# samiazirar/mvtracker

Hardware: AMD Instinct MI355X
Metric: query-points*frames/sec, 4-view 24-frame 512x512 @1024 queries (higher is better)
Workload: dtype bf16; 1 GPU; c3: 4-view synthetic 24-frame 512x512, 1024 queries, bf16 (configs[2], the metric's config); 4-view 24-frame 512x512, 1024 queries per GPU, corr K=16 x 4 levels, iters=4, 3 windows, random-init weights (seeded recipe); queries_total=1024, parallelism=query-shard x1, frame_store=bf16 rows

## Files before the change

mvtracker_amd/csrc/attention_mfma.hip:

```cpp
#include "common.h"

namespace {

typedef __bf16 bf16x8 __attribute__((ext_vector_type(8)));
typedef __bf16 bf16x4 __attribute__((ext_vector_type(4)));
typedef unsigned u32x2 __attribute__((ext_vector_type(2)));
typedef unsigned u32x4 __attribute__((ext_vector_type(4)));

constexpr int DH = 48;
constexpr int LDV = 40;

__device__ __forceinline__ bf16x8 load8(const float* base, long long off, int bf) {
  if (bf) return __builtin_bit_cast(bf16x8, *reinterpret_cast<const u32x4*>(reinterpret_cast<const unsigned short*>(base) + off));
  const float* p = base + off;
  const f32x4 a = *reinterpret_cast<const f32x4*>(p), b = *reinterpret_cast<const f32x4*>(p + 4);
  const bf16x4 x = __builtin_convertvector(a, bf16x4), y = __builtin_convertvector(b, bf16x4);
  bf16x8 o;
#pragma unroll
  for (int e = 0; e < 4; ++e) {
    o[e] = x[e];
    o[4 + e] = y[e];
  }
  return o;
}

template <int KS, bool BFIN>
__device__ __forceinline__ void attention_mfma(const float* __restrict__ q, int ldq, long long q_gs, long long q_is,
                                               const float* __restrict__ k, const float* __restrict__ v, int ldkv, long long k_gs,
                                               long long k_is, float* __restrict__ o, int ldo, int groups, int nq, int nk, int heads,
                                               int bf_out, float* __restrict__ ws, unsigned bx, unsigned by, unsigned gx, unsigned gy) {
  constexpr int bf_in = BFIN ? 1 : 0;
  constexpr int NW = KS == 1 ? 4 : KS;
  constexpr int VT = 64 * LDV;
  constexpr int MERGE = KS > 1 ? (KS - 1) * 64 * 68 : 0;
  __shared__ __attribute__((aligned(16))) unsigned short vts[NW * VT];
  __shared__ float red[MERGE > 0 ? MERGE : 1];
  const int lane = threadIdx.x & 63;
  const int wave = __builtin_amdgcn_readfirstlane(threadIdx.x >> 6);
  const int r = lane & 31, h = lane >> 5;
  unsigned short* vt = vts + wave * VT;

  const int chunks = (nq + 63) / 64;
  const long long nchunk = (long long)groups * heads * chunks;
  unsigned bxl = bx, byl = by;
#ifndef MVT_ATTN_NO_XCD
  if (KS > 1 && ws) {
    const unsigned total = gx * gy;
    if (total % 8 == 0) {
      const unsigned L = bx + gx * by;
      const unsigned V = (L % 8) * (total / 8) + L / 8;
      bxl = V / gy;
      byl = V % gy;
    }
  }
#endif
  const long long chunk_id = KS == 1 ? (long long)bxl * 4 + wave : (long long)bxl;
  const bool chunk_ok = chunk_id < nchunk;
  const long long cid = chunk_ok ? chunk_id : 0;
  const int qc = (int)(cid % chunks);
  const int hd = (int)((cid / chunks) % heads);
  const long long g = cid / ((long long)chunks * heads);

  const int nkb = (nk + 31) / 32;
  const int gper = ws ? (nkb + (int)gy - 1) / (int)gy : nkb;
  const int g0 = ws ? (int)byl * gper : 0;
  const int g1 = g0 + gper < nkb ? g0 + gper : nkb;
  const int per = (gper + KS - 1) / KS;
  const int kb0 = KS == 1 ? g0 : g0 + wave * per;
  const int kb1 = KS == 1 ? g1 : (kb0 + per < g1 ? kb0 + per : g1);
  const long long kvbase = (g * k_gs) * ldkv + hd * DH;
  const long long kstep = k_is * ldkv;
  struct KV {
    bf16x8 kf[3];
    f32x4 vraw[6];
  };
  auto load_kv = [&](int kb, KV& t) {
    const int key = kb * 32 + r;
    const long long ko = kvbase + (long long)(key < nk ? key : nk - 1) * kstep;
#pragma unroll
    for (int ks = 0; ks < 3; ++ks) t.kf[ks] = load8(k, ko + ks * 16 + 8 * h, bf_in);
    const long long vo = ko + 24 * h;
#pragma unroll
    for (int i = 0; i < 6; ++i) {
      if (bf_in) {
        const uint2 w = *reinterpret_cast<const uint2*>(reinterpret_cast<const unsigned short*>(v) + vo + 4 * i);
        t.vraw[i] = (f32x4){__uint_as_float(w.x), __uint_as_float(w.y), 0.f, 0.f};
      } else {
        t.vraw[i] = *reinterpret_cast<const f32x4*>(v + vo + 4 * i);
      }
    }
  };
  KV cur;
  if (kb0 < kb1) load_kv(kb0, cur);

  const float scale = 1.0f / sqrtf((float)DH);
  bf16x8 qf[2][3];
#pragma unroll
  for (int mb = 0; mb < 2; ++mb) {
    const int qi = qc * 64 + mb * 32 + r;
    const long long qo = (g * q_gs + (long long)(qi < nq ? qi : nq - 1) * q_is) * ldq + hd * DH;
#pragma unroll
    for (int ks = 0; ks < 3; ++ks) {
      f32x4 a = load_act4(q, qo + ks * 16 + 8 * h, bf_in), b = load_act4(q, qo + ks * 16 + 8 * h + 4, bf_in);
#pragma unroll
      for (int e = 0; e < 4; ++e) {
        a[e] *= scale;
        b[e] *= scale;
      }
      const bf16x4 x = __builtin_convertvector(a, bf16x4), y = __builtin_convertvector(b, bf16x4);
#pragma unroll
      for (int e = 0; e < 4; ++e) {
        qf[mb][ks][e] = x[e];
        qf[mb][ks][4 + e] = y[e];
      }
    }
  }
  for (int i = lane; i < 16 * LDV; i += 64) vt[48 * LDV + i] = 0;
  __builtin_amdgcn_fence(__ATOMIC_SEQ_CST, "wavefront");

  f32x16 oacc[2][2];
  float m[2], l[2];
#pragma unroll
  for (int mb = 0; mb < 2; ++mb) {
    m[mb] = -INFINITY;
    l[mb] = 0.f;
#pragma unroll
    for (int db = 0; db < 2; ++db)
#pragma unroll
      for (int e = 0; e < 16; ++e) oacc[mb][db][e] = 0.f;
  }

#pragma unroll 1
  for (int kb = kb0; kb < kb1; ++kb) {
    KV nxt = cur;
    if (kb + 1 < kb1) load_kv(kb + 1, nxt);
    const int key = kb * 32 + r;
    bf16x8 kf[3];
#pragma unroll
    for (int ks = 0; ks < 3; ++ks) kf[ks] = cur.kf[ks];
    {
      __builtin_amdgcn_fence(__ATOMIC_SEQ_CST, "wavefront");
#pragma unroll
      for (int i = 0; i < 6; ++i) {
        f32x4 a = cur.vraw[i];
        if (bf_in) {
          const unsigned wx = __float_as_uint(a[0]), wy = __float_as_uint(a[1]);
          a = (f32x4){__uint_as_float(wx << 16), __uint_as_float(wx & 0xFFFF0000u), __uint_as_float(wy << 16), __uint_as_float(wy & 0xFFFF0000u)};
        }
        if (key >= nk) a = (f32x4){0.f, 0.f, 0.f, 0.f};
        const u32x2 w = __builtin_bit_cast(u32x2, __builtin_convertvector(a, bf16x4));
#pragma unroll
        for (int e = 0; e < 4; ++e) vt[(24 * h + 4 * i + e) * LDV + r] = (unsigned short)((e & 1) ? (w[e >> 1] >> 16) : (w[e >> 1] & 0xFFFFu));
      }
      __builtin_amdgcn_fence(__ATOMIC_SEQ_CST, "wavefront");
    }
#pragma unroll
    for (int mb = 0; mb < 2; ++mb) {
      f32x16 s;
#pragma unroll
      for (int e = 0; e < 16; ++e) s[e] = 0.f;
#pragma unroll
      for (int ks = 0; ks < 3; ++ks) s = __builtin_amdgcn_mfma_f32_32x32x16_bf16(kf[ks], qf[mb][ks], s, 0, 0, 0);
      float mx = -INFINITY;
#pragma unroll
      for (int e = 0; e < 16; ++e) {
        const int kk = kb * 32 + (e & 3) + 8 * (e >> 2) + 4 * h;
        if (kk >= nk) s[e] = -INFINITY;
        mx = fmaxf(mx, s[e]);
      }
      mx = fmaxf(mx, __shfl_xor(mx, 32, 64));
      const float mn = fmaxf(m[mb], mx);
      const float corr = (m[mb] == -INFINITY) ? 0.f : __expf(m[mb] - mn);
      float ps = 0.f;
#pragma unroll
      for (int e = 0; e < 16; ++e) {
        s[e] = __expf(s[e] - mn);
        ps += s[e];
      }
      l[mb] = l[mb] * corr + ps;
      m[mb] = mn;
      if (__ballot(corr != 1.0f)) {
#pragma unroll
        for (int db = 0; db < 2; ++db)
#pragma unroll
          for (int e = 0; e < 16; ++e) oacc[mb][db][e] *= corr;
      }
#pragma unroll
      for (int sk = 0; sk < 2; ++sk) {
        f32x4 lo4, hi4;
#pragma unroll
        for (int e = 0; e < 4; ++e) {
          lo4[e] = s[8 * sk + e];
          hi4[e] = s[8 * sk + 4 + e];
        }
        const bf16x4 bl = __builtin_convertvector(lo4, bf16x4), bh = __builtin_convertvector(hi4, bf16x4);
        bf16x8 pb;
#pragma unroll
        for (int e = 0; e < 4; ++e) {
          pb[e] = bl[e];
          pb[4 + e] = bh[e];
        }
#pragma unroll
        for (int db = 0; db < 2; ++db) {
          const unsigned short* vr = &vt[(db * 32 + r) * LDV + 16 * sk + 4 * h];
          const u32x2 a0 = *reinterpret_cast<const u32x2*>(vr), a1 = *reinterpret_cast<const u32x2*>(vr + 8);
          const bf16x8 va = __builtin_bit_cast(bf16x8, (u32x4){a0[0], a0[1], a1[0], a1[1]});
          oacc[mb][db] = __builtin_amdgcn_mfma_f32_32x32x16_bf16(va, pb, oacc[mb][db], 0, 0, 0);
        }
      }
    }
    cur = nxt;
  }

  if (KS > 1) {
    if (wave > 0) {
      float* rr = red + ((wave - 1) * 64 + lane) * 68;
#pragma unroll
      for (int mb = 0; mb < 2; ++mb) {
        rr[mb] = m[mb];
        rr[2 + mb] = l[mb];
#pragma unroll
        for (int db = 0; db < 2; ++db)
#pragma unroll
          for (int e = 0; e < 16; ++e) rr[4 + (mb * 2 + db) * 16 + e] = oacc[mb][db][e];
      }
    }
    __syncthreads();
    if (wave > 0) return;
#pragma unroll 1
    for (int w = 0; w < KS - 1; ++w) {
      const float* rr = red + (w * 64 + lane) * 68;
#pragma unroll
      for (int mb = 0; mb < 2; ++mb) {
        const float mw = rr[mb];
        const float mn = fmaxf(m[mb], mw);
        const float ca = (m[mb] == -INFINITY) ? 0.f : __expf(m[mb] - mn);
        const float cb = (mw == -INFINITY) ? 0.f : __expf(mw - mn);
        l[mb] = fmaf(l[mb], ca, rr[2 + mb] * cb);
#pragma unroll
        for (int db = 0; db < 2; ++db)
#pragma unroll
          for (int e = 0; e < 16; ++e) oacc[mb][db][e] = fmaf(oacc[mb][db][e], ca, rr[4 + (mb * 2 + db) * 16 + e] * cb);
        m[mb] = mn;
      }
    }
  }
  if (!chunk_ok) return;
  if (ws) {
    {
      const long long rec = byl * nchunk + chunk_id;
      *reinterpret_cast<f32x4*>(ws + mvt_part_off(rec, 0, lane)) = (f32x4){m[0], m[1], l[0], l[1]};
#pragma unroll
      for (int mb = 0; mb < 2; ++mb)
#pragma unroll
        for (int db = 0; db < 2; ++db)
#pragma unroll
          for (int gq = 0; gq < 4; ++gq)
            *reinterpret_cast<f32x4*>(ws + mvt_part_off(rec, 1 + (mb * 2 + db) * 4 + gq, lane)) =
                (f32x4){oacc[mb][db][4 * gq], oacc[mb][db][4 * gq + 1], oacc[mb][db][4 * gq + 2], oacc[mb][db][4 * gq + 3]};
    }
    return;
  }
#pragma unroll
  for (int mb = 0; mb < 2; ++mb) {
    const float lt = l[mb] + __shfl_xor(l[mb], 32, 64);
    const float inv = 1.0f / lt;
    const int qi = qc * 64 + mb * 32 + r;
    if (qi >= nq) continue;
    const long long oo = (g * q_gs + (long long)qi * q_is) * ldo + hd * DH;
#pragma unroll
    for (int db = 0; db < 2; ++db) {
#pragma unroll
      for (int gq = 0; gq < 4; ++gq) {
        const int d = db * 32 + 8 * gq + 4 * h;
        if (d < DH) {
          f32x4 t;
#pragma unroll
          for (int e = 0; e < 4; ++e) t[e] = oacc[mb][db][4 * gq + e] * inv;
          store_act4(o, oo + d, t, bf_out);
        }
      }
    }
  }
}

__device__ __forceinline__ void attention_merge(const float* __restrict__ ws, int nsplit, long long nchunk, long long q_gs, long long q_is,
                                                float* __restrict__ o, int ldo, int nq, int heads, int bf_out, long long bid) {
  const int lane = threadIdx.x & 63;
  const long long cid = bid * 4 + (threadIdx.x >> 6);
  if (cid >= nchunk) return;
  const int r = lane & 31, h = lane >> 5;
  const int chunks = (nq + 63) / 64;
  const int qc = (int)(cid % chunks);
  const int hd = (int)((cid / chunks) % heads);
  const long long g = cid / ((long long)chunks * heads);
  float m[2], l[2];
  f32x16 oacc[2][2];
  auto ld = [&](long long rec, int quad) { return *reinterpret_cast<const f32x4*>(ws + mvt_part_off(rec, quad, lane)); };
  {
    const f32x4 q0 = ld(cid, 0);
#pragma unroll
    for (int mb = 0; mb < 2; ++mb) {
      m[mb] = q0[mb];
      l[mb] = q0[2 + mb];
#pragma unroll
      for (int db = 0; db < 2; ++db)
#pragma unroll
        for (int gq = 0; gq < 4; ++gq) {
          const f32x4 t = ld(cid, 1 + (mb * 2 + db) * 4 + gq);
#pragma unroll
          for (int e = 0; e < 4; ++e) oacc[mb][db][4 * gq + e] = t[e];
        }
    }
  }
#pragma unroll 1
  for (int w = 1; w < nsplit; ++w) {
    const long long rec = w * nchunk + cid;
    const f32x4 q0 = ld(rec, 0);
#pragma unroll
    for (int mb = 0; mb < 2; ++mb) {
      const float mw = q0[mb];
      const float mn = fmaxf(m[mb], mw);
      const float ca = (m[mb] == -INFINITY) ? 0.f : __expf(m[mb] - mn);
      const float cb = (mw == -INFINITY) ? 0.f : __expf(mw - mn);
      l[mb] = fmaf(l[mb], ca, q0[2 + mb] * cb);
#pragma unroll
      for (int db = 0; db < 2; ++db)
#pragma unroll
        for (int gq = 0; gq < 4; ++gq) {
          const f32x4 t = ld(rec, 1 + (mb * 2 + db) * 4 + gq);
#pragma unroll
          for (int e = 0; e < 4; ++e) oacc[mb][db][4 * gq + e] = fmaf(oacc[mb][db][4 * gq + e], ca, t[e] * cb);
        }
      m[mb] = mn;
    }
  }
#pragma unroll
  for (int mb = 0; mb < 2; ++mb) {
    const float lt = l[mb] + __shfl_xor(l[mb], 32, 64);
    const float inv = 1.0f / lt;
    const int qi = qc * 64 + mb * 32 + r;
    if (qi >= nq) continue;
    const long long oo = (g * q_gs + (long long)qi * q_is) * ldo + hd * DH;
#pragma unroll
    for (int db = 0; db < 2; ++db) {
#pragma unroll
      for (int gq = 0; gq < 4; ++gq) {
        const int d = db * 32 + 8 * gq + 4 * h;
        if (d < DH) {
          f32x4 t;
#pragma unroll
          for (int e = 0; e < 4; ++e) t[e] = oacc[mb][db][4 * gq + e] * inv;
          store_act4(o, oo + d, t, bf_out);
        }
      }
    }
  }
}

#define ATTN_ARGS                                                                                                               \
  const float *__restrict__ q, int ldq, long long q_gs, long long q_is, const float *__restrict__ k, const float *__restrict__ v, \
      int ldkv, long long k_gs, long long k_is, float *__restrict__ o, int ldo, int groups
template <int KS, bool BFIN>
__global__ __launch_bounds__(KS == 1 ? 256 : KS * 64) void attention_mfma_kernel(ATTN_ARGS, int nq, int nk, int heads, int bf_in_unused,
                                                                                int bf_out, float* __restrict__ ws) {
  attention_mfma<KS, BFIN>(q, ldq, q_gs, q_is, k, v, ldkv, k_gs, k_is, o, ldo, groups, nq, nk, heads, bf_out, ws, blockIdx.x, blockIdx.y,
                           gridDim.x, gridDim.y);
}
__global__ __launch_bounds__(256) void attention_merge_kernel(const float* __restrict__ ws, int nsplit, long long nchunk, long long q_gs,
                                                              long long q_is, float* __restrict__ o, int ldo, int nq, int heads,
                                                              int bf_out) {
  attention_merge(ws, nsplit, nchunk, q_gs, q_is, o, ldo, nq, heads, bf_out, blockIdx.x);
}

__device__ __forceinline__ const float* row_ptr(const float* base, long long r, int ld, int bf) {
  return bf ? reinterpret_cast<const float*>(reinterpret_cast<const unsigned short*>(base) + r * ld) : base + r * ld;
}

template <int KS, bool BFIN>
__global__ __launch_bounds__(KS == 1 ? 256 : KS * 64) void attention_mfma_seg_kernel(ATTN_ARGS, int heads, int bf_out,
                                                                                    float* __restrict__ ws, mvt_seg_table t) {
  const int s = mvt_seg_find(t, blockIdx.x);
  const int bf = BFIN ? 1 : 0;
  attention_mfma<KS, BFIN>(row_ptr(q, t.qrow[s], ldq, bf), ldq, q_gs, q_is, row_ptr(k, t.krow[s], ldkv, bf), row_ptr(v, t.krow[s], ldkv, bf),
                           ldkv, k_gs, k_is, const_cast<float*>(row_ptr(o, t.qrow[s], ldo, bf_out)), ldo, groups, t.nq[s], t.nk[s], heads,
                           bf_out, ws ? ws + t.ws[s] : nullptr, (unsigned)(blockIdx.x - t.blk[s]), blockIdx.y,
                           (unsigned)(t.blk[s + 1] - t.blk[s]), gridDim.y);
}
__global__ __launch_bounds__(256) void attention_merge_seg_kernel(const float* __restrict__ ws, int nsplit, int groups, long long q_gs,
                                                                  long long q_is, float* __restrict__ o, int ldo, int heads, int bf_out,
                                                                  mvt_seg_table t) {
  const int s = mvt_seg_find(t, blockIdx.x);
  const long long nchunk = (long long)groups * heads * ((t.nq[s] + 63) / 64);
  attention_merge(ws + t.ws[s], nsplit, nchunk, q_gs, q_is, const_cast<float*>(row_ptr(o, t.qrow[s], ldo, bf_out)), ldo, t.nq[s], heads,
                  bf_out, blockIdx.x - t.blk[s]);
}
#undef ATTN_ARGS

}

extern "C" int mvt_attention_bf16(const void* q, int ldq, long long q_gs, long long q_is, const void* k, const void* v,
                                  int ldkv, long long k_gs, long long k_is, void* o, int ldo, int groups, int nq, int nk,
                                  int heads, int dh, int io_flags, float* workspace, void* stream) {
  MVT_REQUIRE((io_flags & ~(MVT_IO_IN_BF16 | MVT_IO_OUT_BF16 | MVT_ATTN_PARTIALS_ONLY)) == 0);
  const bool partials_only = (io_flags & MVT_ATTN_PARTIALS_ONLY) != 0;
  const int bf_in = io_flags & MVT_IO_IN_BF16 ? 1 : 0, bf_out = io_flags & MVT_IO_OUT_BF16 ? 1 : 0;
  MVT_REQUIRE(!bf_in || (ldq % 8 == 0 && ldkv % 8 == 0));
  MVT_REQUIRE(!bf_out || ldo % 8 == 0);
  MVT_REQUIRE(q && k && v && o && groups > 0 && nq > 0 && nk > 0 && heads > 0 && dh == DH);
  MVT_REQUIRE(ldq % 4 == 0 && ldkv % 4 == 0 && ldo % 4 == 0 && ldq >= heads * dh && ldkv >= heads * dh && ldo >= heads * dh);
  MVT_REQUIRE(((uintptr_t)q % 16 == 0) && ((uintptr_t)k % 16 == 0) && ((uintptr_t)v % 16 == 0) && ((uintptr_t)o % 16 == 0));
  const long long nchunk = (long long)groups * heads * ((nq + 63) / 64);
#define LAUNCH_T(KS, BF, BLOCKS, THREADS, WSP)                                                                                        \
  hipLaunchKernelGGL((attention_mfma_kernel<KS, BF>), BLOCKS, dim3(THREADS), 0, mvt_stream(stream), (const float*)q, ldq, q_gs, q_is, \
                     (const float*)k, (const float*)v, ldkv, k_gs, k_is, (float*)o, ldo, groups, nq, nk, heads, bf_in, bf_out, WSP)
#define LAUNCH(KS, BLOCKS, THREADS)                                         \
  do {                                                                      \
    if (bf_in) LAUNCH_T(KS, true, dim3((unsigned)(BLOCKS)), THREADS, WS);  \
    else LAUNCH_T(KS, false, dim3((unsigned)(BLOCKS)), THREADS, WS);       \
  } while (0)
  constexpr int NSPLIT = MVT_ATTN_NSPLIT;
  MVT_REQUIRE(!partials_only || (nk >= 512 && nchunk < 256 && workspace && ((nk + 31) / 32) % NSPLIT == 0));
  if (nk >= 512 && nchunk < 256 && workspace && ((nk + 31) / 32) % NSPLIT == 0) {
    MVT_REQUIRE((uintptr_t)workspace % 16 == 0);
#define WS workspace
    if (bf_in) LAUNCH_T(4, true, dim3((unsigned)nchunk, NSPLIT), 256, workspace);
    else LAUNCH_T(4, false, dim3((unsigned)nchunk, NSPLIT), 256, workspace);
#undef WS
    if (!partials_only)
      hipLaunchKernelGGL(attention_merge_kernel, dim3((unsigned)mvt_cdiv(nchunk, 4)), dim3(256), 0, mvt_stream(stream), workspace, NSPLIT,
                         nchunk, q_gs, q_is, (float*)o, ldo, nq, heads, bf_out);
    return mvt_launch_status();
  }
#define WS nullptr
  if (nk >= 512 && nchunk < 1024) {
    LAUNCH(4, nchunk, 256);
  } else {
    LAUNCH(1, mvt_cdiv(nchunk, 4), 256);
  }
#undef WS
#undef LAUNCH
#undef LAUNCH_T
  return mvt_launch_status();
}

extern "C" int mvt_attention_bf16_segmented(const void* q, int ldq, long long q_gs, long long q_is, const void* k, const void* v, int ldkv,
                                            long long k_gs, long long k_is, void* o, int ldo, int groups, int heads, int dh, int io_flags,
                                            int nseg, const long long* q_row0, const int* nq, const long long* k_row0, const int* nk,
                                            float* workspace, long long ws_floats, void* stream) {
  MVT_REQUIRE((io_flags & ~(MVT_IO_IN_BF16 | MVT_IO_OUT_BF16)) == 0);
  const int bf_in = io_flags & MVT_IO_IN_BF16 ? 1 : 0, bf_out = io_flags & MVT_IO_OUT_BF16 ? 1 : 0;
  MVT_REQUIRE(!bf_in || (ldq % 8 == 0 && ldkv % 8 == 0));
  MVT_REQUIRE(!bf_out || ldo % 8 == 0);
  MVT_REQUIRE(q && k && v && o && groups > 0 && heads > 0 && dh == DH && nseg > 0 && q_row0 && nq && k_row0 && nk);
  MVT_REQUIRE(ldq % 4 == 0 && ldkv % 4 == 0 && ldo % 4 == 0 && ldq >= heads * dh && ldkv >= heads * dh && ldo >= heads * dh);
  MVT_REQUIRE(((uintptr_t)q % 16 == 0) && ((uintptr_t)k % 16 == 0) && ((uintptr_t)v % 16 == 0) && ((uintptr_t)o % 16 == 0));
  MVT_REQUIRE(!workspace || ((uintptr_t)workspace % 16 == 0 && ws_floats >= 0));
  constexpr int NSPLIT = MVT_ATTN_NSPLIT;
  auto form_of = [&](int s, long long* blocks) {
    const long long nchunk = (long long)groups * heads * ((nq[s] + 63) / 64);
    if (nk[s] >= 512 && nchunk < 256 && workspace && ((nk[s] + 31) / 32) % NSPLIT == 0) {
      *blocks = nchunk;
      return 0;
    }
    *blocks = nk[s] >= 512 && nchunk < 1024 ? nchunk : mvt_cdiv(nchunk, 4);
    return nk[s] >= 512 && nchunk < 1024 ? 1 : 2;
  };
  long long ws_need = 0;
  for (int s = 0; s < nseg; ++s) {
    MVT_REQUIRE(nq[s] > 0 && nk[s] > 0 && q_row0[s] >= 0 && k_row0[s] >= 0);
    long long nb;
    if (form_of(s, &nb) == 0) ws_need += (long long)NSPLIT * nb * MVT_PART_FLOATS;
  }
  MVT_REQUIRE(ws_need <= ws_floats || ws_need == 0);
  long long ws_next = 0;
  for (int form = 0; form < 3; ++form) {
    mvt_seg_table t, tm;
    t.n = tm.n = 0;
    t.blk[0] = tm.blk[0] = 0;
    for (int s = 0; s <= nseg; ++s) {
      long long nb = 0;
      if (s < nseg && form_of(s, &nb) == form) {
        const int i = t.n;
        t.nq[i] = tm.nq[i] = nq[s];
        t.nk[i] = tm.nk[i] = nk[s];
        t.qrow[i] = tm.qrow[i] = q_row0[s];
        t.krow[i] = tm.krow[i] = k_row0[s];
        t.ws[i] = tm.ws[i] = form == 0 ? ws_next : 0;
        if (form == 0) ws_next += (long long)NSPLIT * nb * MVT_PART_FLOATS;
        t.blk[i + 1] = t.blk[i] + nb;
        tm.blk[i + 1] = tm.blk[i] + mvt_cdiv(nb, 4);
        t.n = tm.n = i + 1;
      }
      if (t.n == 0 || (t.n < MVT_SEG_MAX && s < nseg)) continue;
      const unsigned blocks = (unsigned)t.blk[t.n];
#define LAUNCH_SEG(KS, BF, GRID, THREADS, WSP)                                                                                  \
  hipLaunchKernelGGL((attention_mfma_seg_kernel<KS, BF>), GRID, dim3(THREADS), 0, mvt_stream(stream), (const float*)q, ldq, q_gs, \
                     q_is, (const float*)k, (const float*)v, ldkv, k_gs, k_is, (float*)o, ldo, groups, heads, bf_out, WSP, t)
      if (form == 0) {
        if (bf_in) LAUNCH_SEG(4, true, dim3(blocks, NSPLIT), 256, workspace);
        else LAUNCH_SEG(4, false, dim3(blocks, NSPLIT), 256, workspace);
        hipLaunchKernelGGL(attention_merge_seg_kernel, dim3((unsigned)tm.blk[tm.n]), dim3(256), 0, mvt_stream(stream), workspace, NSPLIT,
                           groups, q_gs, q_is, (float*)o, ldo, heads, bf_out, tm);
      } else if (form == 1) {
        if (bf_in) LAUNCH_SEG(4, true, dim3(blocks), 256, nullptr);
        else LAUNCH_SEG(4, false, dim3(blocks), 256, nullptr);
      } else {
        if (bf_in) LAUNCH_SEG(1, true, dim3(blocks), 256, nullptr);
        else LAUNCH_SEG(1, false, dim3(blocks), 256, nullptr);
      }
#undef LAUNCH_SEG
      t.n = tm.n = 0;
    }
  }
  return mvt_launch_status();
}
```

mvtracker_amd/csrc/common.h:

```cpp
#pragma once
#include <hip/hip_runtime.h>
#include <stdint.h>

#include "../../include/mvtracker_hip.h"

typedef float f32x4 __attribute__((ext_vector_type(4)));
typedef float f32x16 __attribute__((ext_vector_type(16)));

#define MVT_WAVE 64

#define MVT_REQUIRE(cond) \
  do {                    \
    if (!(cond)) return MVT_ERR_ARG; \
  } while (0)

static inline int mvt_launch_status() {
  hipError_t e = hipGetLastError();
  return e == hipSuccess ? MVT_OK : MVT_ERR_HIP_BASE + (int)e;
}

static inline hipStream_t mvt_stream(void* s) { return (hipStream_t)s; }

static inline long long mvt_cdiv(long long a, long long b) { return (a + b - 1) / b; }

static inline bool mvt_frame_small_tiles(long long ntok, long long S) { return ntok * S >= 4096 && mvt_cdiv(ntok, 32) * S <= 256; }

__device__ __forceinline__ float mvt_gelu_tanh(float x) {
  const float k2 = 2.0f * 0.7978845608028654f * (x + 0.044715f * x * x * x);
  return x * __builtin_amdgcn_rcpf(1.0f + __expf(-k2));
}

__device__ __forceinline__ float mvt_gelu_erf(float x) { return 0.5f * x * (1.0f + erff(x * 0.7071067811865476f)); }

__device__ __forceinline__ float mvt_act(float x, int act) {
  switch (act) {
    case MVT_ACT_RELU: return fmaxf(x, 0.0f);
    case MVT_ACT_GELU_TANH: return mvt_gelu_tanh(x);
    case MVT_ACT_GELU_ERF: return mvt_gelu_erf(x);
    default: return x;
  }
}

__device__ __forceinline__ f32x4 mvt_unproject_point(const float* __restrict__ K, const float* __restrict__ E, int x, int y, float st, float d) {
  float px = ((float)x + 0.5f) * st - 0.5f, py = ((float)y + 0.5f) * st - 0.5f;
  float cx = (K[0] * px + K[1] * py + K[2]) * d;
  float cy = (K[3] * px + K[4] * py + K[5]) * d;
  float cz = (K[6] * px + K[7] * py + K[8]) * d;
  f32x4 o;
  o[0] = E[0] * cx + E[1] * cy + E[2] * cz + E[3];
  o[1] = E[4] * cx + E[5] * cy + E[6] * cz + E[7];
  o[2] = E[8] * cx + E[9] * cy + E[10] * cz + E[11];
  o[3] = 0.f;
  return o;
}

__device__ __forceinline__ unsigned short mvt_bf16_bits(float v) { return __builtin_bit_cast(unsigned short, (__bf16)v); }
__device__ __forceinline__ f32x4 load_act4(const float* base, long long off, int is_bf16) {
  if (!is_bf16) return *reinterpret_cast<const f32x4*>(base + off);
  const uint2 w = *reinterpret_cast<const uint2*>(reinterpret_cast<const unsigned short*>(base) + off);
  return (f32x4){__uint_as_float(w.x << 16), __uint_as_float(w.x & 0xFFFF0000u), __uint_as_float(w.y << 16),
                 __uint_as_float(w.y & 0xFFFF0000u)};
}
__device__ __forceinline__ void store_act(float* base, long long off, float v, int is_bf16) {
  if (!is_bf16) base[off] = v;
  else reinterpret_cast<unsigned short*>(base)[off] = mvt_bf16_bits(v);
}
__device__ __forceinline__ void store_act4(float* base, long long off, const f32x4& v, int is_bf16) {
  if (!is_bf16) {
    *reinterpret_cast<f32x4*>(base + off) = v;
  } else {
    uint2 w;
    w.x = (unsigned)mvt_bf16_bits(v[0]) | ((unsigned)mvt_bf16_bits(v[1]) << 16);
    w.y = (unsigned)mvt_bf16_bits(v[2]) | ((unsigned)mvt_bf16_bits(v[3]) << 16);
    *reinterpret_cast<uint2*>(reinterpret_cast<unsigned short*>(base) + off) = w;
  }
}

#define MVT_PART_FLOATS (17 * 64 * 4)
__device__ __forceinline__ long long mvt_part_off(long long rec, int quad, int lane) { return (rec * 17 + quad) * 256 + lane * 4; }

#define MVT_SEG_MAX 32
struct mvt_seg_table {
  int n;
  int nq[MVT_SEG_MAX], nk[MVT_SEG_MAX];
  long long qrow[MVT_SEG_MAX], krow[MVT_SEG_MAX], ws[MVT_SEG_MAX];
  long long blk[MVT_SEG_MAX + 1];
};
__device__ __forceinline__ int mvt_seg_find(const mvt_seg_table& t, long long b) {
  int s = 0;
  while (s + 1 < t.n && b >= t.blk[s + 1]) ++s;
  return s;
}

__device__ __forceinline__ float wave_sum(float v) {
#pragma unroll
  for (int o = 32; o > 0; o >>= 1) v += __shfl_xor(v, o, 64);
  return v;
}

__device__ __forceinline__ float wave_max(float v) {
#pragma unroll
  for (int o = 32; o > 0; o >>= 1) v = fmaxf(v, __shfl_xor(v, o, 64));
  return v;
}

__device__ __forceinline__ unsigned long long shfl_xor_u64(unsigned long long v, int o) {
  unsigned lo = (unsigned)v, hi = (unsigned)(v >> 32);
  lo = __shfl_xor(lo, o, 64);
  hi = __shfl_xor(hi, o, 64);
  return ((unsigned long long)hi << 32) | lo;
}

__device__ __forceinline__ unsigned long long wave_min_u64(unsigned long long v) {
#pragma unroll
  for (int o = 32; o > 0; o >>= 1) {
    unsigned long long w = shfl_xor_u64(v, o);
    v = w < v ? w : v;
  }
  return v;
}

__device__ __forceinline__ double wave_sum_f64(double v) {
#pragma unroll
  for (int o = 32; o > 0; o >>= 1) v += __shfl_xor(v, o, 64);
  return v;
}

__device__ __forceinline__ double block_sum_f64(double v, double* s_red) {
  v = wave_sum_f64(v);
  __syncthreads();
  if ((threadIdx.x & 63) == 0) s_red[threadIdx.x >> 6] = v;
  __syncthreads();
  return (s_red[0] + s_red[1]) + (s_red[2] + s_red[3]);
}

__device__ __forceinline__ double& st_f64(long long* state, int w) { return reinterpret_cast<double*>(state)[w]; }
__device__ __forceinline__ double st_f64(const long long* state, int w) { return reinterpret_cast<const double*>(state)[w]; }
```

Baseline: 1.075 million query-points*frames/s.

## Add 512-thread split-K attention kernel with per-wave 32-query tiles and double-buffered V

Adds a new bf16 split-K attention kernel that uses 8 waves per workgroup: four key-split groups, each with two waves owning 32-query halves, instead of 4 waves each handling 64 queries. V^T tiles are staged into double-buffered LDS images shared by the wave pair, and K/V loads are prefetched two blocks ahead, with workgroup barriers per iteration. The merge of partial softmax states runs through LDS and m/l are exchanged across the pair before writing partials. It is the default for bf16 input, with an env flag to return to the old kernel, and includes optional timestamp instrumentation compiled out by default. Per-iteration barriers and larger LDS footprint may reduce occupancy.

Result: no change. 1.079 million query-points*frames/s, median of 2 (+0.4%).

```diff
diff --git a/mvtracker_amd/csrc/attention_mfma.hip b/mvtracker_amd/csrc/attention_mfma.hip
--- a/mvtracker_amd/csrc/attention_mfma.hip
+++ b/mvtracker_amd/csrc/attention_mfma.hip
@@ -22,6 +22,36 @@
     o[4 + e] = y[e];
   }
   return o;
+}
+
+#ifdef MVT_STAMPS
+__device__ unsigned long long mvt_attn_stamp_buf[2 * 8 * 64];
+#ifndef MVT_STAMP_WG1
+#define MVT_STAMP_WG1 40
+#endif
+#define STAMP_IF(sel, i)                                                                \
+  do {                                                                                  \
+    __builtin_amdgcn_sched_barrier(0);                                                  \
+    unsigned long long t_;                                                              \
+    asm volatile("s_memtime %0\n\ts_waitcnt lgkmcnt(0)" : "=s"(t_)::"memory");          \
+    __builtin_amdgcn_sched_barrier(0);                                                  \
+    if (lane == 0 && (sel) && (bxl == 0 || bxl == MVT_STAMP_WG1) && byl == 0)           \
+      mvt_attn_stamp_buf[((bxl ? 1 : 0) * 8 + wave) * 64 + (i)] = t_;                   \
+  } while (0)
+#define STAMP_LANDED() asm volatile("s_waitcnt vmcnt(0)" ::: "memory")
+#else
+#define STAMP_IF(sel, i) \
+  do {                   \
+  } while (0)
+#define STAMP_LANDED() \
+  do {                 \
+  } while (0)
+#endif
+
+__device__ __forceinline__ void lds_barrier() {
+  __builtin_amdgcn_fence(__ATOMIC_RELEASE, "workgroup", "local");
+  __builtin_amdgcn_s_barrier();
+  __builtin_amdgcn_fence(__ATOMIC_ACQUIRE, "workgroup", "local");
 }
 
 template <int KS, bool BFIN>
@@ -54,6 +84,8 @@
     }
   }
 #endif
+#define STAMP(i) STAMP_IF(KS > 1 && BFIN && ws != nullptr, i)
+  STAMP(0);
   const long long chunk_id = KS == 1 ? (long long)bxl * 4 + wave : (long long)bxl;
   const bool chunk_ok = chunk_id < nchunk;
   const long long cid = chunk_ok ? chunk_id : 0;
@@ -115,6 +147,9 @@
       }
     }
   }
+  STAMP(1);
+  STAMP_LANDED();
+  STAMP(2);
   for (int i = lane; i < 16 * LDV; i += 64) vt[48 * LDV + i] = 0;
   __builtin_amdgcn_fence(__ATOMIC_SEQ_CST, "wavefront");
 
@@ -154,6 +189,7 @@
       }
       __builtin_amdgcn_fence(__ATOMIC_SEQ_CST, "wavefront");
     }
+    if (kb - kb0 < 8) STAMP(3 + 3 * (kb - kb0));
 #pragma unroll
     for (int mb = 0; mb < 2; ++mb) {
       f32x16 s;
@@ -208,6 +244,7 @@
           oacc[mb][db] = __builtin_amdgcn_mfma_f32_32x32x16_bf16(va, pb, oacc[mb][db], 0, 0, 0);
         }
       }
+      if (kb - kb0 < 8) STAMP(4 + 3 * (kb - kb0) + mb);
     }
     cur = nxt;
   }
@@ -225,7 +262,9 @@
           for (int e = 0; e < 16; ++e) rr[4 + (mb * 2 + db) * 16 + e] = oacc[mb][db][e];
       }
     }
+    STAMP(40);
     __syncthreads();
+    STAMP(41);
     if (wave > 0) return;
 #pragma unroll 1
     for (int w = 0; w < KS - 1; ++w) {
@@ -244,6 +283,7 @@
         m[mb] = mn;
       }
     }
+    STAMP(42);
   }
   if (!chunk_ok) return;
   if (ws) {
@@ -259,6 +299,8 @@
             *reinterpret_cast<f32x4*>(ws + mvt_part_off(rec, 1 + (mb * 2 + db) * 4 + gq, lane)) =
                 (f32x4){oacc[mb][db][4 * gq], oacc[mb][db][4 * gq + 1], oacc[mb][db][4 * gq + 2], oacc[mb][db][4 * gq + 3]};
     }
+    STAMP_LANDED();
+    STAMP(43);
     return;
   }
 #pragma unroll
@@ -282,6 +324,245 @@
       }
     }
   }
+}
+#undef STAMP
+
+constexpr int Q32_VT = 64 * LDV;
+constexpr int Q32_RED = 3 * 2 * 34 * 64;
+static_assert(4 * 2 * Q32_VT * 2 <= Q32_RED * 4, "the merge records cover the eight V^T images");
+__global__ __launch_bounds__(512) void attention_mfma_q32_kernel(const unsigned short* __restrict__ q, int ldq, long long q_gs,
+                                                                 long long q_is, const unsigned short* __restrict__ k,
+                                                                 const unsigned short* __restrict__ v, int ldkv, long long k_gs,
+                                                                 long long k_is, int groups, int nq, int nk, int heads,
+                                                                 float* __restrict__ ws) {
+  __shared__ __attribute__((aligned(16))) float smem[Q32_RED + 128];
+  float* red = smem;
+  float* xch = smem + Q32_RED;
+  const int lane = threadIdx.x & 63;
+  const int wave = __builtin_amdgcn_readfirstlane(threadIdx.x >> 6);
+  const int kq = wave >> 1, mb = wave & 1;
+  const int r = lane & 31, h = lane >> 5;
+  unsigned short* img = reinterpret_cast<unsigned short*>(smem) + kq * 2 * Q32_VT;
+
+  const int chunks = (nq + 63) / 64;
+  const long long nchunk = (long long)groups * heads * chunks;
+  const unsigned gx = gridDim.x, gy = gridDim.y;
+  unsigned bxl = blockIdx.x, byl = blockIdx.y;
+#ifndef MVT_ATTN_NO_XCD
+  {
+    const unsigned total = gx * gy;
+    if (total % 8 == 0) {
+      const unsigned L = blockIdx.x + gx * blockIdx.y;
+      const unsigned V = (L % 8) * (total / 8) + L / 8;
+      bxl = V / gy;
+      byl = V % gy;
+    }
+  }
+#endif
+#define STAMP(i) STAMP_IF(true, i)
+  STAMP(0);
+  const long long cid = bxl;
+  const int qc = (int)(cid % chunks);
+  const int hd = (int)((cid / chunks) % heads);
+  const long long g = cid / ((long long)chunks * heads);
+
+  const int nkb = (nk + 31) / 32;
+  const int gper = (nkb + (int)gy - 1) / (int)gy;
+  const int g0 = (int)byl * gper;
+  const int g1 = g0 + gper < nkb ? g0 + gper : nkb;
+  const int per = (gper + 3) / 4;
+  const int kb0 = g0 + kq * per;
+  const int kb1 = kb0 + per < g1 ? kb0 + per : g1;
+  const int nb = kb1 > kb0 ? kb1 - kb0 : 0;
+  const long long kvbase = (g * k_gs) * ldkv + hd * DH;
+  const long long kstep = k_is * ldkv;
+  struct KV {
+    bf16x8 kf[3];
+    u32x2 vw[3];
+  };
+  auto load_kv = [&](int kb, KV& t) {
+    const int key = kb * 32 + r;
+    const long long ko = kvbase + (long long)(key < nk ? key : nk - 1) * kstep;
+#pragma unroll
+    for (int ks = 0; ks < 3; ++ks) t.kf[ks] = __builtin_bit_cast(bf16x8, *reinterpret_cast<const u32x4*>(k + ko + ks * 16 + 8 * h));
+#pragma unroll
+    for (int i = 0; i < 3; ++i) t.vw[i] = *reinterpret_cast<const u32x2*>(v + ko + 24 * h + 12 * mb + 4 * i);
+  };
+  auto stage_v = [&](int kb, const KV& t, unsigned short* im) {
+    const bool live = kb * 32 + r < nk;
+#pragma unroll
+    for (int i = 0; i < 3; ++i) {
+      const u32x2 w = live ? t.vw[i] : (u32x2){0u, 0u};
+#pragma unroll
+      for (int e = 0; e < 4; ++e)
+        im[(24 * h + 12 * mb + 4 * i + e) * LDV + r] = (unsigned short)((e & 1) ? (w[e >> 1] >> 16) : (w[e >> 1] & 0xFFFFu));
+    }
+  };
+  KV a, b;
+  if (nb > 0) load_kv(kb0, a);
+
+  const float scale = 1.0f / sqrtf((float)DH);
+  u32x4 qraw[3];
+  {
+    const int qi = qc * 64 + mb * 32 + r;
+    const long long qo = (g * q_gs + (long long)(qi < nq ? qi : nq - 1) * q_is) * ldq + hd * DH;
+#pragma unroll
+    for (int ks = 0; ks < 3; ++ks) qraw[ks] = *reinterpret_cast<const u32x4*>(q + qo + ks * 16 + 8 * h);
+  }
+  if (nb > 1) load_kv(kb0 + 1, b);
+  bf16x8 qf[3];
+#pragma unroll
+  for (int ks = 0; ks < 3; ++ks) {
+    f32x4 x = (f32x4){__uint_as_float(qraw[ks][0] << 16), __uint_as_float(qraw[ks][0] & 0xFFFF0000u), __uint_as_float(qraw[ks][1] << 16),
+                      __uint_as_float(qraw[ks][1] & 0xFFFF0000u)};
+    f32x4 y = (f32x4){__uint_as_float(qraw[ks][2] << 16), __uint_as_float(qraw[ks][2] & 0xFFFF0000u), __uint_as_float(qraw[ks][3] << 16),
+                      __uint_as_float(qraw[ks][3] & 0xFFFF0000u)};
+#pragma unroll
+    for (int e = 0; e < 4; ++e) {
+      x[e] *= scale;
+      y[e] *= scale;
+    }
+    const bf16x4 xb = __builtin_convertvector(x, bf16x4), yb = __builtin_convertvector(y, bf16x4);
+#pragma unroll
+    for (int e = 0; e < 4; ++e) {
+      qf[ks][e] = xb[e];
+      qf[ks][4 + e] = yb[e];
+    }
+  }
+  STAMP(1);
+#ifdef MVT_STAMPS
+  STAMP_LANDED();
+  STAMP(2);
+#endif
+  {
+    unsigned* z = reinterpret_cast<unsigned*>(img + mb * Q32_VT + 48 * LDV);
+    for (int i = lane; i < 16 * LDV / 2; i += 64) z[i] = 0u;
+  }
+  if (nb > 0) stage_v(kb0, a, img);
+
+  f32x16 oacc[2];
+  float m = -INFINITY, l = 0.f;
+#pragma unroll
+  for (int db = 0; db < 2; ++db)
+#pragma unroll
+    for (int e = 0; e < 16; ++e) oacc[db][e] = 0.f;
+
+#pragma unroll 1
+  for (int it = 0; it < per; ++it) {
+    lds_barrier();
+    if (it < 8) STAMP(3 + 3 * it);
+    if (it >= nb) continue;
+    const int kb = kb0 + it;
+    const unsigned short* vt = img + (it & 1) * Q32_VT;
+    f32x16 s;
+#pragma unroll
+    for (int e = 0; e < 16; ++e) s[e] = 0.f;
+#pragma unroll
+    for (int ks = 0; ks < 3; ++ks) s = __builtin_amdgcn_mfma_f32_32x32x16_bf16(a.kf[ks], qf[ks], s, 0, 0, 0);
+    float mx = -INFINITY;
+#pragma unroll
+    for (int e = 0; e < 16; ++e) {
+      const int kk = kb * 32 + (e & 3) + 8 * (e >> 2) + 4 * h;
+      if (kk >= nk) s[e] = -INFINITY;
+      mx = fmaxf(mx, s[e]);
+    }
+    mx = fmaxf(mx, __shfl_xor(mx, 32, 64));
+    const float mn = fmaxf(m, mx);
+    const float corr = (m == -INFINITY) ? 0.f : __expf(m - mn);
+    float ps = 0.f;
+#pragma unroll
+    for (int e = 0; e < 16; ++e) {
+      s[e] = __expf(s[e] - mn);
+      ps += s[e];
+    }
+    l = l * corr + ps;
+    m = mn;
+    if (__ballot(corr != 1.0f)) {
+#pragma unroll
+      for (int db = 0; db < 2; ++db)
+#pragma unroll
+        for (int e = 0; e < 16; ++e) oacc[db][e] *= corr;
+    }
+#pragma unroll
+    for (int sk = 0; sk < 2; ++sk) {
+      f32x4 lo4, hi4;
+#pragma unroll
+      for (int e = 0; e < 4; ++e) {
+        lo4[e] = s[8 * sk + e];
+        hi4[e] = s[8 * sk + 4 + e];
+      }
+      const bf16x4 bl = __builtin_convertvector(lo4, bf16x4), bh = __builtin_convertvector(hi4, bf16x4);
+      bf16x8 pb;
+#pragma unroll
+      for (int e = 0; e < 4; ++e) {
+        pb[e] = bl[e];
+        pb[4 + e] = bh[e];
+      }
+#pragma unroll
+      for (int db = 0; db < 2; ++db) {
+        const unsigned short* vr = &vt[(db * 32 + r) * LDV + 16 * sk + 4 * h];
+        const u32x2 a0 = *reinterpret_cast<const u32x2*>(vr), a1 = *reinterpret_cast<const u32x2*>(vr + 8);
+        const bf16x8 va = __builtin_bit_cast(bf16x8, (u32x4){a0[0], a0[1], a1[0], a1[1]});
+        oacc[db] = __builtin_amdgcn_mfma_f32_32x32x16_bf16(va, pb, oacc[db], 0, 0, 0);
+      }
+    }
+    if (it < 8) STAMP(4 + 3 * it);
+    if (it + 1 < nb) {
+      stage_v(kb + 1, b, img + ((it + 1) & 1) * Q32_VT);
+#pragma unroll
+      for (int ks = 0; ks < 3; ++ks) a.kf[ks] = b.kf[ks];
+      if (it + 2 < nb) load_kv(kb + 2, b);
+      if (it < 8) STAMP(5 + 3 * it);
+    }
+  }
+
+  lds_barrier();
+  if (kq > 0) {
+    float* rr = red + ((kq - 1) * 2 + mb) * 34 * 64 + lane;
+    rr[0] = m;
+    rr[64] = l;
+#pragma unroll
+    for (int db = 0; db < 2; ++db)
+#pragma unroll
+      for (int e = 0; e < 16; ++e) rr[(2 + db * 16 + e) * 64] = oacc[db][e];
+  }
+  STAMP(40);
+  lds_barrier();
+  STAMP(41);
+  if (kq == 0) {
+#pragma unroll 1
+    for (int w = 0; w < 3; ++w) {
+      const float* rr = red + (w * 2 + mb) * 34 * 64 + lane;
+      const float mw = rr[0];
+      const float mn = fmaxf(m, mw);
+      const float ca = (m == -INFINITY) ? 0.f : __expf(m - mn);
+      const float cb = (mw == -INFINITY) ? 0.f : __expf(mw - mn);
+      l = fmaf(l, ca, rr[64] * cb);
+#pragma unroll
+      for (int db = 0; db < 2; ++db)
+#pragma unroll
+        for (int e = 0; e < 16; ++e) oacc[db][e] = fmaf(oacc[db][e], ca, rr[(2 + db * 16 + e) * 64] * cb);
+      m = mn;
+    }
+    if (mb == 1) {
+      xch[lane] = m;
+      xch[64 + lane] = l;
+    }
+  }
+  STAMP(42);
+  lds_barrier();
+  if (kq > 0) return;
+  const long long rec = byl * nchunk + cid;
+  if (mb == 0) *reinterpret_cast<f32x4*>(ws + mvt_part_off(rec, 0, lane)) = (f32x4){m, xch[lane], l, xch[64 + lane]};
+#pragma unroll
+  for (int db = 0; db < 2; ++db)
+#pragma unroll
+    for (int gq = 0; gq < 4; ++gq)
+      *reinterpret_cast<f32x4*>(ws + mvt_part_off(rec, 1 + (mb * 2 + db) * 4 + gq, lane)) =
+          (f32x4){oacc[db][4 * gq], oacc[db][4 * gq + 1], oacc[db][4 * gq + 2], oacc[db][4 * gq + 3]};
+  STAMP_LANDED();
+  STAMP(43);
+#undef STAMP
 }
 
 __device__ __forceinline__ void attention_merge(const float* __restrict__ ws, int nsplit, long long nchunk, long long q_gs, long long q_is,
@@ -398,6 +679,18 @@
 #undef ATTN_ARGS
 
 }
+
+#ifdef MVT_STAMPS
+extern "C" int mvt_debug_read_attn_stamps(unsigned long long* host) {
+  return hipMemcpyFromSymbol(host, HIP_SYMBOL(mvt_attn_stamp_buf), sizeof(unsigned long long) * 2 * 8 * 64) == hipSuccess ? MVT_OK : MVT_ERR_HIP_BASE;
+}
+extern "C" int mvt_debug_clear_attn_stamps() {
+  static unsigned long long z[2 * 8 * 64];
+  return hipMemcpyToSymbol(HIP_SYMBOL(mvt_attn_stamp_buf), z, sizeof(z)) == hipSuccess ? MVT_OK : MVT_ERR_HIP_BASE;
+}
+#endif
+
+static inline int attn_wave64q_switch() { return mvt_env_flag("MVT_ATTN_WAVE64Q"); }
 
 extern "C" int mvt_attention_bf16(const void* q, int ldq, long long q_gs, long long q_is, const void* k, const void* v,
                                   int ldkv, long long k_gs, long long k_is, void* o, int ldo, int groups, int nq, int nk,
@@ -424,7 +717,10 @@
   if (nk >= 512 && nchunk < 256 && workspace && ((nk + 31) / 32) % NSPLIT == 0) {
     MVT_REQUIRE((uintptr_t)workspace % 16 == 0);
 #define WS workspace
-    if (bf_in) LAUNCH_T(4, true, dim3((unsigned)nchunk, NSPLIT), 256, workspace);
+    if (bf_in && !attn_wave64q_switch())
+      hipLaunchKernelGGL(attention_mfma_q32_kernel, dim3((unsigned)nchunk, NSPLIT), dim3(512), 0, mvt_stream(stream), (const unsigned short*)q,
+                         ldq, q_gs, q_is, (const unsigned short*)k, (const unsigned short*)v, ldkv, k_gs, k_is, groups, nq, nk, heads, workspace);
+    else if (bf_in) LAUNCH_T(4, true, dim3((unsigned)nchunk, NSPLIT), 256, workspace);
     else LAUNCH_T(4, false, dim3((unsigned)nchunk, NSPLIT), 256, workspace);
 #undef WS
     if (!partials_only)
diff --git a/mvtracker_amd/csrc/common.h b/mvtracker_amd/csrc/common.h
--- a/mvtracker_amd/csrc/common.h
+++ b/mvtracker_amd/csrc/common.h
@@ -1,6 +1,7 @@
 #pragma once
 #include <hip/hip_runtime.h>
 #include <stdint.h>
+#include <stdlib.h>
 
 #include "../../include/mvtracker_hip.h"
 
@@ -22,6 +23,11 @@
 static inline hipStream_t mvt_stream(void* s) { return (hipStream_t)s; }
 
 static inline long long mvt_cdiv(long long a, long long b) { return (a + b - 1) / b; }
+
+static inline int mvt_env_flag(const char* name) {
+  const char* e = getenv(name);
+  return e && atoi(e) != 0;
+}
 
 static inline bool mvt_frame_small_tiles(long long ntok, long long S) { return ntok * S >= 4096 && mvt_cdiv(ntok, 32) * S <= 256; }
 
```
